# AIGC-Audio/AudioGPT

Measured on AMD Instinct MI355X. Metric: generated audio-seconds/sec (10s clip, 100 DDIM steps) [3 independent batches of 8 prompts in flight per GPU], higher is better.
Workload: dtype bf16x3; 1 GPU; Make-An-Audio T2A batch=8/GPU, 100 DDIM steps, CFG 1.5, UNet+VAE+HiFi-GAN(16k), fp32 storage, bf16x3-split MFMA (hi/lo, fp32 accumulate; meets the fp32 parity gates); prompts_per_gpu=8, ddim_steps=100, mel_frames=624, hipgraph=True, batches_in_flight=3, cfg_lanes=1, concurrency_hint=3, parallelism=prompt-sharded x1 (RCCL bcast cond / gather wav)

## Files before the change

### audiogpt_amd/csrc/ddim.cpp

```cpp
#include "models.h"

#include <cmath>
#include <cstdio>
#include <cstring>

#ifdef MAA_ROCTX
#include <roctracer/roctx.h>
#define MAA_RANGE_PUSH(name) roctxRangePushA(name)
#define MAA_RANGE_POP() roctxRangePop()
#else
#define MAA_RANGE_PUSH(name) ((void)0)
#define MAA_RANGE_POP() ((void)0)
#endif

namespace maa {

namespace {

struct Loop {
    Ctx& ctx;
    UNet& unet;
    const maa_ddim_args& a;
    bool concat, cfg, masked, logging, emb_hoist, share, split;
    int nB, Cin;
// ... 80 lines not shown
        h_step = start;
        MAA_HIP(hipMemcpyAsync(d_step, &h_step, 4, hipMemcpyHostToDevice, ctx.stream));

        if (emb_hoist) unet.emb_table(ctx, tab_t, a.S, emb_tab);

        if (!concat && a.d_cond) {
            if (cfg)
                unet.set_context_cfg(ctx, a.d_uncond, a.d_cond, a.B, a.L, crops);
            else
                unet.set_context(ctx, a.d_cond, nB, a.L, crops);
        }

        const bool two_lanes = cfg && ctx.split_cfg();
        lane2 = two_lanes ? &side_lane(ctx) : nullptr;
        if (lane2 && ctx.prof && !lane2->prof) {
            lane2->prof = new Profiler;
            lane2->prof->detail = ctx.prof->detail;
        }
        share = cfg && emb_hoist && ctx.tune.cfg_shared;
    }

    void prepare() {
        launch_ddim_prepare(ctx, xs, concat ? ccs : nullptr, a.B, nB, per, per_in - per, tab_t, tab_coef, d_step, xin, cur_t,
                            cur_coef, a.d_mask, a.d_x0, a.d_noise_q, a.S, emb_hoist ? emb_tab : nullptr, (int)emb_w, cur_emb, rows);
    }

    void forward() {
        const float* in = xin;
        float* out = eps;
        int h = a.H, w = a.W;
        if (split) {
            launch_split_unfold(ctx, xin, nB, Cin, a.H, a.W, a.split_kh, a.split_kw, a.split_sh, a.split_sw, zin);
            in = zin, out = ecrop, h = a.split_kh, w = a.split_kw;
        }
        const int half = a.B * crops;
        if (lane2) {
            MAA_HIP(hipEventRecord(ctx.ev_fork, ctx.stream));
            MAA_HIP(hipStreamWaitEvent(lane2->stream, ctx.ev_fork, 0));
            unet.forward(ctx, in, cur_t, unet.context_ptr, half, h, w, out, emb_hoist ? cur_emb : nullptr, 0, share ? 2 : 0);
            unet.forward(*lane2, in + (size_t)half * per_crop_in, cur_t + half, unet.context_ptr, half, h, w,
                         out + (size_t)half * per_crop, emb_hoist ? cur_emb : nullptr, half, share ? 3 : 0);
            MAA_HIP(hipEventRecord(ctx.ev_join, lane2->stream));
            MAA_HIP(hipStreamWaitEvent(ctx.stream, ctx.ev_join, 0));
        } else
            unet.forward(ctx, in, cur_t, unet.context_ptr, rows, h, w, out, emb_hoist ? cur_emb : nullptr, -1, share ? 1 : 0);
        if (split)
            launch_split_fold(ctx, ecrop, wT, norm, nB, a.C, a.H, a.W, a.split_kh, a.split_kw, a.split_sh, a.split_sw, eps);
    }

    std::vector<unsigned long long> key(const float* noise_p) const {
        std::vector<unsigned long long> k;
        unet.graph_key(k);
        unsigned scale_bits, temp_bits;
        static_assert(sizeof(scale_bits) == sizeof(a.scale), "float bits");
        std::memcpy(&scale_bits, &a.scale, 4);
        std::memcpy(&temp_bits, &a.temperature, 4);
        k.push_back(temp_bits);
        for (unsigned long long v : {(unsigned long long)a.S, (unsigned long long)a.B, (unsigned long long)a.C, (unsigned long long)a.H,
                                     (unsigned long long)a.W, (unsigned long long)a.Cc, (unsigned long long)a.L,
                                     (unsigned long long)cfg, (unsigned long long)concat, (unsigned long long)scale_bits,
                                     (unsigned long long)ctx.dtype, (unsigned long long)reinterpret_cast<uintptr_t>(slab),
                                     (unsigned long long)reinterpret_cast<uintptr_t>(a.d_mask),
                                     (unsigned long long)reinterpret_cast<uintptr_t>(a.d_x0),
                                     (unsigned long long)reinterpret_cast<uintptr_t>(a.d_noise_q),
                                     (unsigned long long)reinterpret_cast<uintptr_t>(a.h_sigmas ? noise_p : nullptr),
                                     (unsigned long long)reinterpret_cast<uintptr_t>(logging ? a.d_log_x : nullptr),
                                     (unsigned long long)reinterpret_cast<uintptr_t>(logging ? a.d_log_x0 : nullptr),
                                     (unsigned long long)(a.h_sigmas ? 1 : 0),
                                     (unsigned long long)reinterpret_cast<uintptr_t>(ctx.stream),
                                     (unsigned long long)reinterpret_cast<uintptr_t>(ctx.ws.base()),
                                     (unsigned long long)ctx.ws.capacity(),
                                     (unsigned long long)reinterpret_cast<uintptr_t>(lane2 ? lane2->stream : nullptr),
                                     (unsigned long long)reinterpret_cast<uintptr_t>(lane2 ? lane2->ws.base() : nullptr),
                                     (unsigned long long)(lane2 ? lane2->ws.capacity() : 0),
                                     (unsigned long long)a.split_kh, (unsigned long long)a.split_kw, (unsigned long long)a.split_sh,
                                     (unsigned long long)a.split_sw, (unsigned long long)reinterpret_cast<uintptr_t>(wT)})
            k.push_back(v);
        return k;
    }
};

template <class F>
void capture_step(Ctx& ctx, StepGraph& sg, F&& body, std::vector<unsigned long long> key) {
    MAA_HIP(hipStreamBeginCapture(ctx.stream, hipStreamCaptureModeRelaxed));
    try {
        body();
    } catch (...) {
        hipGraph_t dead = nullptr;
        (void)hipStreamEndCapture(ctx.stream, &dead);
        if (dead) (void)hipGraphDestroy(dead);
        throw;
    }
    MAA_HIP(hipStreamEndCapture(ctx.stream, &sg.graph));
    MAA_HIP(hipGraphInstantiate(&sg.exec, sg.graph, nullptr, nullptr, 0));
    sg.key = std::move(key);
}

void ddim_run(Ctx& ctx, UNet& unet, const maa_ddim_args& a, int start, int n_steps, const float* noise_p, float* d_x) {
    MAA_CHECK(a.S > 0 && a.B > 0, "ddim: empty problem");
    MAA_CHECK(start >= 0 && start < a.S && n_steps > 0 && n_steps <= start + 1, "ddim: steps outside the schedule");
    Loop lp(ctx, unet, a, start, d_x);

    auto step_body = [&]() {
        lp.prepare();
        lp.forward();
        launch_ddim_step(ctx, lp.xin, lp.per, lp.per_in, lp.eps, lp.cfg ? lp.eps + a.B * lp.per : nullptr, a.scale, lp.cur_coef,
                         (long long)a.B * lp.per, lp.xs, a.h_sigmas ? noise_p : nullptr, a.temperature, a.S,
                         lp.logging ? a.d_log_x : nullptr, lp.logging ? a.d_log_x0 : nullptr, lp.d_step);
    };

    StepGraph& sg = ctx.ddim_graph;
    int first = 0;
    if (a.use_graph && sg.exec && sg.key == lp.key(noise_p)) {
    } else if (a.use_graph) {
        sg.clear();
        step_body();
        first = 1;
        if (n_steps > 1) capture_step(ctx, sg, step_body, lp.key(noise_p));
    }
    for (int i = first; i < n_steps; ++i) {
#ifdef MAA_ROCTX
        char range[48];
        std::snprintf(range, sizeof(range), "ddim_step %d/%d t=%d", i + 1, n_steps, (int)a.h_timesteps[start - i]);
#endif
        MAA_RANGE_PUSH(range);
        if (a.use_graph)
            MAA_HIP(hipGraphLaunch(sg.exec, ctx.stream));
        else
            step_body();
        MAA_RANGE_POP();
    }
    MAA_HIP(hipMemcpyAsync(d_x, lp.xs, (size_t)a.B * lp.per * 4, hipMemcpyDeviceToDevice, ctx.stream));
    MAA_HIP(hipStreamSynchronize(ctx.stream));
}

}

void ddim_sample(Ctx& ctx, UNet& unet, const maa_ddim_args& a, float* d_x) { ddim_run(ctx, unet, a, a.S - 1, a.S, a.d_noise_p, d_x); }

void ddim_decode(Ctx& ctx, UNet& unet, const maa_ddim_args& a, int t_start, float* d_x) {
    MAA_CHECK(a.S > 0 && a.B > 0, "ddim_decode: empty problem");
    MAA_CHECK(t_start >= 0 && t_start <= a.S, "ddim_decode: t_start must lie in [0, S]");
    MAA_CHECK(!a.d_mask && !a.d_x0 && !a.d_noise_q && !a.h_sqrt_ac && !a.h_sqrt_1mac,
              "ddim_decode: decode has no mask / x0 (ddim.py:243-245)");
    MAA_CHECK(a.n_log == 0 && !a.d_log_x && !a.d_log_x0, "ddim_decode: decode logs no intermediates");
    if (t_start == 0) return;
    const float* noise_p = nullptr;
    if (a.h_sigmas && a.d_noise_p) {
        const long long n = (long long)a.B * a.C * a.H * a.W;
        noise_p = reinterpret_cast<const float*>(reinterpret_cast<uintptr_t>(a.d_noise_p) -
                                                 (uintptr_t)((long long)(a.S - t_start) * n * (long long)sizeof(float)));
    }
    ddim_run(ctx, unet, a, t_start - 1, t_start, noise_p, d_x);
}

void ldm_plms_sample(Ctx& ctx, UNet& unet, const maa_ddim_args& a, float* d_x) {
    MAA_CHECK(a.S > 0 && a.B > 0, "plms: empty problem");
    MAA_CHECK(!a.h_sigmas && !a.d_noise_p, "plms: ddim_eta must be 0 for PLMS (no sigmas, no step noise)");
    Loop lp(ctx, unet, a, a.S - 1, d_x);
    const long long n = (long long)a.B * lp.per;
    float* ring = static_cast<float*>(ctx.plms_ring.get((size_t)3 * n * sizeof(float), ctx.stream));
    const float* eps_c = lp.cfg ? lp.eps + n : nullptr;
    float* log_x = lp.logging ? a.d_log_x : nullptr;
    float* log_x0 = lp.logging ? a.d_log_x0 : nullptr;

    auto euler_step = [&]() {
        lp.prepare();
        lp.forward();
        launch_ldm_plms_euler_mid(ctx, lp.xin, lp.per, lp.per_in, a.B, lp.nB, lp.eps, eps_c, a.scale, lp.cur_coef, lp.xs, ring,
                                  lp.tab_t, lp.cur_t, lp.emb_hoist ? lp.emb_tab : nullptr, (int)lp.emb_w, lp.cur_emb, lp.rows);
        lp.forward();
        launch_ldm_plms_euler_final(ctx, lp.eps, eps_c, a.scale, lp.cur_coef, n, lp.xs, ring, log_x, log_x0, lp.d_step);
    };
    auto ab_step = [&]() {
        lp.prepare();
        lp.forward();
// ... 193 lines not shown
```

### audiogpt_amd/csrc/igemm_dma2.hip

```cpp
#include "igemm_epilogue.h"

#include <cstdio>
#include <cstdlib>
#include <cstring>
#include <type_traits>

namespace maa {

namespace {

template <int BM, int BN, int WGM, int WGN, int NS, int TERMS>
__global__ __launch_bounds__(64 * WGM * WGN) void igemm_dma2_kernel(const IGemm p, int ntiles, int tiles, int Nb,
                                                                     int cps, int items, float* __restrict__ part) {
    constexpr int NW = WGM * WGN, NTH = 64 * NW;
    constexpr int WTM = BM / WGM, WTN = BN / WGN;
    constexpr int MI = WTM / 32, NI = WTN / 32;
    constexpr int ROWS = BM + BN;
    constexpr int STAGE = ROWS * 128;
    constexpr int AI = BM / 8 / NW, BI = BN / 8 / NW;
    constexpr int IPW = AI + BI;
    static_assert(BM % (8 * NW) == 0 && BN % (8 * NW) == 0 && NW % 2 == 0, "copy assignment");
    static_assert(WTM % 32 == 0 && WTN % 32 == 0 && BM % 32 == 0, "tile");
    static_assert(NS >= 3 && (NS - 2) * IPW <= 63, "stages / vmcnt field");
    extern __shared__ __attribute__((aligned(1024))) char smem[];
// ... 157 lines not shown
        }
#pragma unroll
        for (int i = 0; i < MI; ++i)
#pragma unroll
            for (int j = 0; j < NI; ++j) acc[i][j] = __builtin_amdgcn_mfma_f32_32x32x16_bf16(f.ah[i], f.bh[j], acc[i][j], 0, 0, 0);
    };

    int c_w = w_first, c_rem = 0;
    auto item_chunks = [&](int w) __attribute__((always_inline)) {
        const int slice = (w_lo + w) / tiles;
        return min(nchunks, (slice + 1) * cps) - slice * cps;
    };
    auto finish_item = [&]() __attribute__((always_inline)) {
        const int item = w_lo + c_w;
        const int slice = item / tiles, tile = item - slice * tiles;
        const int mt = tile / ntiles, nt = tile - mt * ntiles;
        if (part == nullptr) {
            igemm_epilogue<MI, NI>(p, acc, mt * BM + wm * WTM, nt * BN + wn * WTN, lrow, lk, 0, Nb, rpb);
        } else {
            float* pp = part + ((long long)item * (MI * NI * 4) * NTH + tid) * 4;
#pragma unroll
            for (int i = 0; i < MI; ++i)
#pragma unroll
                for (int j = 0; j < NI; ++j)
#pragma unroll
                    for (int q = 0; q < 4; ++q) {
                        const f32x4 v = {acc[i][j][4 * q], acc[i][j][4 * q + 1], acc[i][j][4 * q + 2], acc[i][j][4 * q + 3]};
                        *reinterpret_cast<f32x4*>(pp + (long long)((i * NI + j) * 4 + q) * NTH * 4) = v;
                    }
        }
        zero_acc();
        c_w += w_step;
        if (c_w >= w_cnt) return false;
        c_rem = item_chunks(c_w);
        return true;
    };

    setup_item(g_w);
    c_rem = item_chunks(c_w);
#pragma unroll
    for (int s = 0; s < NS - 1; ++s) issue(s);

    {
        wait_vmcnt<(NS - 2) * IPW>();
        __builtin_amdgcn_s_barrier();
        Frags f0, f1;
        read_frags(smem, 0, f0);
        int st = 0;
        for (;;) {
            const char* cur = smem + st * STAGE;
            const int st_next = st + 1 == NS ? 0 : st + 1;
            const int st_fill = st == 0 ? NS - 1 : st - 1;
            read_frags(cur, 1, f1);
            __builtin_amdgcn_sched_barrier(0);
            mma(f0);
            __builtin_amdgcn_sched_barrier(0);
            wait_vmcnt<(NS - 3) * IPW>();
            __builtin_amdgcn_s_barrier();
            read_frags(smem + st_next * STAGE, 0, f0);
            __builtin_amdgcn_sched_barrier(0);
            static_for<0, TERMS * MI * NI>([&](auto xc) {
                constexpr int x = decltype(xc)::value;
                constexpr int t = x / (MI * NI) + (3 - TERMS), i = (x % (MI * NI)) / NI, j = x % NI;
                if constexpr (t == 0)
                    acc[i][j] = __builtin_amdgcn_mfma_f32_32x32x16_bf16(f1.al[i], f1.bh[j], acc[i][j], 0, 0, 0);
                else if constexpr (t == 1)
                    acc[i][j] = __builtin_amdgcn_mfma_f32_32x32x16_bf16(f1.ah[i], f1.bl[j], acc[i][j], 0, 0, 0);
                else
                    acc[i][j] = __builtin_amdgcn_mfma_f32_32x32x16_bf16(f1.ah[i], f1.bh[j], acc[i][j], 0, 0, 0);
                if constexpr (x < IPW) copy1(st_fill, xc);
                __builtin_amdgcn_sched_barrier(0);
            });
            if constexpr (IPW > TERMS * MI * NI)
                static_for<TERMS * MI * NI, IPW>([&](auto jc) { copy1(st_fill, jc); });
            advance();
            st = st_next;
            if (--c_rem == 0)
                if (!finish_item()) break;
        }
    }
    wait_vmcnt<0>();
}

template <int JW, int MI, int NI, int WGN, int NTH>
__global__ __launch_bounds__(NTH) void splitk_reduce_kernel(const IGemm p, const float* __restrict__ part, int S, int tiles,
                                                           int ntiles, int Nb) {
    constexpr int njb = NI / JW, nblk = MI * njb;
    constexpr int WTM = 32 * MI, WTN = 32 * NI;
    constexpr int BM = WTM * (NTH / 64 / WGN), BN = WTN * WGN;
    constexpr long long slab = (long long)(MI * NI * 4) * NTH * 4;
    const int tid = threadIdx.x, lane = tid & 63, wid = tid >> 6;
    const int wi = xcd_contiguous((int)blockIdx.x, (int)gridDim.x);
    const int tile = wi / nblk, blk = wi - tile * nblk;
    const int i = blk / njb, j = (blk - i * njb) * JW;
    const int mt = tile / ntiles, nt = tile - mt * ntiles;
    const int wm = wid / WGN, wn = wid - wm * WGN;
    f32x16 acc[1][JW];
#pragma unroll
    for (int jj = 0; jj < JW; ++jj) {
        const float* src = part + (long long)tile * slab + ((long long)((i * NI + j + jj) * 4) * NTH + tid) * 4;
        f32x4 v[4];
#pragma unroll
        for (int q = 0; q < 4; ++q) v[q] = *reinterpret_cast<const f32x4*>(src + (long long)q * NTH * 4);
        for (int s = 1; s < S; ++s) {
            const float* sp = src + (long long)s * tiles * slab;
#pragma unroll
            for (int q = 0; q < 4; ++q) v[q] += *reinterpret_cast<const f32x4*>(sp + (long long)q * NTH * 4);
        }
#pragma unroll
        for (int q = 0; q < 4; ++q)
#pragma unroll
            for (int e = 0; e < 4; ++e) acc[0][jj][4 * q + e] = v[q][e];
    }
    const int rpb = p.Hout * p.Wout;
    igemm_epilogue<1, JW>(p, acc, mt * BM + wm * WTM + i * 32, nt * BN + wn * WTN + j * 32, lane & 31, lane >> 5, 0, Nb, rpb);
}

template <int MI, int NI, int WGN, int NTH>
void launch_reduce_geom(const Ctx& ctx, const IGemm& p, const float* part, int S, int tiles, int ntiles, int Nb) {
    auto go = [&](auto kern, int blocks) {
        hipLaunchKernelGGL(kern, dim3((unsigned)blocks), dim3(NTH), 0, ctx.stream, p, part, S, tiles, ntiles, Nb);
    };
    if (p.geglu) {
        if constexpr (NI % 2 == 0)
            go(splitk_reduce_kernel<2, MI, NI, WGN, NTH>, tiles * MI * (NI / 2));
        else
            MAA_CHECK(false, "split-K reduce: GEGLU needs value / gate block pairs inside a wave");
        return;
    }
    go(splitk_reduce_kernel<1, MI, NI, WGN, NTH>, tiles * MI * NI);
}

template <int BM, int BN, int WGM, int WGN, int NS>
void launch_one(const Ctx& ctx, const IGemm& p, int Nb, int S, float* part) {
    constexpr int NW = WGM * WGN, NTH = 64 * NW;
    constexpr int MI = BM / WGM / 32, NI = BN / WGN / 32;
    const int ncols = p.N * (p.geglu ? 2 : 1);
    const int mtiles = (p.M + BM - 1) / BM, ntiles = (ncols + BN - 1) / BN;
    const int tiles = mtiles * ntiles;
    const int nchunks = p.K / BK;
    const int cps = (nchunks + S - 1) / S;
    const int Seff = (nchunks + cps - 1) / cps;
    MAA_CHECK(Seff == S, "split-K plan leaves an empty slice");
    MAA_CHECK(!p.geglu || NI % 2 == 0, "GEGLU needs value / gate block pairs inside a wave");
    constexpr size_t lds = (size_t)NS * (BM + BN) * 128;
    static_assert(lds <= 163840, "LDS per workgroup");
    const long long items = (long long)tiles * S;
    long long grid = items;
    {
        const int per_cu = (int)(163840 / lds) < 32 / NW ? (int)(163840 / lds) : 32 / NW;
        const long long cap = (long long)device_cu_count(ctx.device) * (per_cu < 1 ? 1 : per_cu);
        if (grid > cap) grid = cap;
    }
    auto go = [&](auto kern) {
        ensure_dynamic_lds(reinterpret_cast<const void*>(kern), ctx.device, (int)lds);
        hipLaunchKernelGGL(kern, dim3((unsigned)grid), dim3(NTH), lds, ctx.stream, p, ntiles, tiles, Nb, cps, (int)items,
                           S > 1 ? part : nullptr);
    };
    if (ctx.dtype == 2)
        go(igemm_dma2_kernel<BM, BN, WGM, WGN, NS, 1>);
    else
        go(igemm_dma2_kernel<BM, BN, WGM, WGN, NS, 3>);
    if (S > 1) launch_splitk_reduce(ctx, p, part, S, tiles, ntiles, Nb, BM, BN, WGN, MI, NI, NTH);
}

}

void launch_splitk_reduce(const Ctx& ctx, const IGemm& p, const float* part, int S, int tiles, int ntiles, int Nb, int BM,
                          int BN, int WGN, int MI, int NI, int NTH) {
    MAA_CHECK(BM == 32 * MI * (NTH / 64 / WGN) && BN == 32 * NI * WGN, "split-K reduce: tile and wave geometry disagree");
    if (MI == 1 && NI == 5 && WGN == 1 && NTH == 512)
        launch_reduce_geom<1, 5, 1, 512>(ctx, p, part, S, tiles, ntiles, Nb);
    else if (MI == 2 && NI == 2 && WGN == 2 && NTH == 512)
        launch_reduce_geom<2, 2, 2, 512>(ctx, p, part, S, tiles, ntiles, Nb);
    else if (MI == 2 && NI == 2 && WGN == 2 && NTH == 256)
        launch_reduce_geom<2, 2, 2, 256>(ctx, p, part, S, tiles, ntiles, Nb);
    else
        MAA_CHECK(false, "split-K reduce: no instantiation for this workgroup geometry");
}

bool igemm_dma2_takes(const Ctx& ctx, const IGemm& p, IGemmPlan& pl) {
    const int ncols = p.N * (p.geglu ? 2 : 1);
    int S = 0;
    if (!ctx.tune.dma2.empty()) {
        if (ctx.tune.dma2 == "off") return false;
        int cfg = 0, ns = 4, pipe = 1, s = 1, kmin = 0, kmax = 1 << 30;
        const int k = std::sscanf(ctx.tune.dma2.c_str(), "%d,%d,%d,%d,%d,%d", &cfg, &ns, &pipe, &s, &kmin, &kmax);
        if (k >= 4) {
            if (p.K < kmin) return false;
            if (p.K <= kmax) S = s < 1 ? 1 : s;
        }
    }
    if (S == 0) {
        if (p.K < 2048 || ncols < 128 || p.geglu) return false;
        S = 2;
    }
    pl.engine = IGemmPlan::DMA2;
    pl.cfg = 0;
    pl.S = fit_slices(p.K / BK, S);
    return true;
}

void launch_igemm_dma2(const Ctx& ctx, const IGemm& p, const IGemmPlan& pl, float* part) {
    MAA_CHECK(pl.S == 1 || part != nullptr, "igemm_dma2: split-K needs its slab workspace");
    launch_one<128, 128, 2, 2, 4>(ctx, p, pl.Nb, pl.S, part);
}

}
```

### audiogpt_amd/csrc/igemm_epilogue.h

```cpp
#pragma once
#include "igemm_device.h"
#include "maa_internal.h"

namespace maa {

__device__ __forceinline__ float fast_erff(float x) {
    const float t = fminf(fabsf(x), 4.0f);
    const float s = t * t;
    float r = -5.654105860e-04f;
    r = fmaf(r, s, 4.923277665e-03f);
    r = fmaf(r, s, -2.671638510e-02f);
    r = fmaf(r, s, 1.128036441e-01f);
    r = fmaf(r, s, -3.761234978e-01f);
    r = fmaf(r, s, 1.128379127e+00f);
    const float small = r * t;
    float q = 1.330939039e-05f;
    q = fmaf(q, t, -3.175720346e-04f);
    q = fmaf(q, t, 3.436867598e-03f);
    q = fmaf(q, t, -2.262198592e-02f);
    q = fmaf(q, t, 1.033189800e-01f);
    q = fmaf(q, t, 6.390933195e-01f);
    q = fmaf(q, t, 1.125925949e+00f);
    q = fmaf(q, t, 7.569686250e-04f);
    const float large = 1.0f - __builtin_amdgcn_exp2f(q * -1.4426950408889634f);
// ... 99 lines not shown
                for (int r = 0; r < 16; ++r) {
                    settle(ra[r]);
                    settle(rs[r]);
                    settle(cv[r]);
                }
                float outv[16];
#pragma unroll
                for (int r = 0; r < 16; ++r) {
                    float v = acc[i][j][r] * p.alpha + bias;
                    if (p.rowadd) v += ra[r];
                    if (resp) v += rs[r];
                    outv[r] = v;
                }
                if (p.act != 0) {
#pragma unroll
                    for (int r = 0; r < 16; ++r) {
                        float v = outv[r];
                        if (p.act == 1) v = tanhf(v);
                        else if (p.act == 2) v = fmaxf(v, 0.f);
                        else if (p.act == 3) v = 0.5f * v * (1.f + fast_erff(v * 0.70710678118654752440f));
                        else if (p.act == 4) v = v > 0.f ? v : v * p.act_slope;
                        outv[r] = v;
                    }
                }
#pragma unroll
                for (int r = 0; r < 16; ++r) {
                    float v = outv[r] * p.out_scale;
                    if (p.accumulate && !p.c_split) v += cv[r];
                    outv[r] = v;
                }
                if constexpr (PAIR) {
                    const bool even = (lrow & 1) == 0;
#pragma unroll
                    for (int rp = 0; rp < 8; ++rp) {
                        const float keep = even ? outv[2 * rp] : outv[2 * rp + 1];
                        const float give = even ? outv[2 * rp + 1] : outv[2 * rp];
                        const float got = __builtin_bit_cast(float, __builtin_amdgcn_update_dpp(0, __builtin_bit_cast(int, give), 0xB1, 0xF, 0xF, false));
                        const int r = 2 * rp + (even ? 0 : 1);
                        const int m = mb + (r & 3) + 8 * (r >> 2) + 4 * lk;
                        if (m < p.M) {
                            const f32x2 v2 = even ? f32x2{keep, got} : f32x2{got, keep};
                            *reinterpret_cast<f32x2*>(cp + (long long)m * p.ldc + (n & ~1)) = v2;
                        }
                    }
                } else {
#pragma unroll
                    for (int r = 0; r < 16; ++r) {
                        const int m = mb + (r & 3) + 8 * (r >> 2) + 4 * lk;
                        if (m < p.M) {
                            if (p.c_split)
                                store_split_pair(cp + (long long)m * p.ldc, n, outv[r]);
                            else
                                cp[(long long)m * p.ldc + n] = outv[r];
                            if (p.c2) {
                                const float w = outv[r] > 0.f ? outv[r] : outv[r] * p.c2_slope;
                                store_split_pair(p.c2 + coff + (long long)m * p.ldc2, n, w);
                            }
                        }
                    }
                }
            }
        }
    }
}

template <int MI, int NI>
__device__ __forceinline__ void igemm_epilogue(const IGemm& p, f32x16 (&acc)[MI][NI], int m_base, int n_base, int lrow,
                                               int lk, long long coff, int Nb, int rpb) {
    const bool pair = !p.geglu && !p.c_split && p.c2 == nullptr && (p.N & 1) == 0 && (p.ldc & 1) == 0 && (coff & 1) == 0 &&
                      (reinterpret_cast<uintptr_t>(p.c) & 7) == 0;
    const bool rsel = !(p.rowadd && rpb < 32);
    if (pair && rsel)
        igemm_epilogue_impl<MI, NI, true, true>(p, acc, m_base, n_base, lrow, lk, coff, Nb, rpb);
    else if (pair)
        igemm_epilogue_impl<MI, NI, true, false>(p, acc, m_base, n_base, lrow, lk, coff, Nb, rpb);
    else if (rsel)
        igemm_epilogue_impl<MI, NI, false, true>(p, acc, m_base, n_base, lrow, lk, coff, Nb, rpb);
    else
        igemm_epilogue_impl<MI, NI, false, false>(p, acc, m_base, n_base, lrow, lk, coff, Nb, rpb);
}

enum class Epi : int { GENERIC = 0, PLAIN = 1, SPLIT = 2, GEGLU = 3 };

inline Epi igemm_epi_kind(const IGemm& p) {
    const bool pitches = p.ldc > 0 && p.ldc < (1 << 24) && p.ldr >= 0 && p.ldr < (1 << 24);
    if (!pitches || p.Z != 1 || p.M <= 0 || p.alpha != 1.f || p.out_scale != 1.f || p.rowadd || p.act != 0 || p.accumulate || p.c2)
        return Epi::GENERIC;
    if (p.geglu) return p.res ? Epi::GENERIC : Epi::GEGLU;
    if (p.c_split) return (p.N & 1) == 0 ? Epi::SPLIT : Epi::GENERIC;
    const bool pair = (p.N & 1) == 0 && (p.ldc & 1) == 0 && (reinterpret_cast<uintptr_t>(p.c) & 7) == 0;
    return pair ? Epi::PLAIN : Epi::GENERIC;
}

__device__ __forceinline__ constexpr unsigned frag_row(int r) { return (unsigned)((r & 3) + 8 * (r >> 2)); }

template <int MI, int NI, Epi KIND, bool FULL, bool RES>
__device__ __forceinline__ void igemm_epilogue_fast_body(const IGemm& p, f32x16 (&acc)[MI][NI], int mb0, int nb0, int lrow, int lk,
                                                         int Nb) {
    const bool even = (lrow & 1) == 0;
    const unsigned ldc = (unsigned)p.ldc, ldr = (unsigned)p.ldr;
    const unsigned lane_f32 = 4u * lk * ldc + lrow;
    const unsigned lane_pair = (4u * lk + (even ? 0u : 1u)) * ldc + (lrow & ~1);
    const unsigned lane_split = 4u * lk * ldc + (lrow >> 1) + (even ? 0u : 16u);
    const unsigned lane_res = 4u * lk * ldr + lrow;
    if constexpr (KIND == Epi::GEGLU) {
        static_assert(NI % 2 == 0, "GEGLU pairs a value block with a gate block");
#pragma unroll
        for (int i = 0; i < MI; ++i) {
            const int mb = mb0 + i * 32;
            if (!FULL && mb >= p.M) break;
#pragma unroll
            for (int j = 0; j < NI; j += 2) {
                const int cb = nb0 + j * 32, ob = (cb >> 6) * 32;
                const int cpk = cb + lrow;
                if (FULL || (cpk + 32 < Nb && ob + lrow < p.N)) {
                    float bv = p.bias ? p.bias[cpk] : 0.f;
                    float bg = p.bias ? p.bias[cpk + 32] : 0.f;
                    settle(bv);
                    settle(bg);
                    float outv[16];
#pragma unroll
                    for (int r = 0; r < 16; ++r) {
                        const float val = acc[i][j][r] + bv;
                        const float g = acc[i][j + 1][r] + bg;
                        const float gl = 0.5f * g * (1.f + fast_erff(g * 0.70710678118654752440f));
                        outv[r] = val * gl;
                    }
                    float* blk = p.c + ((long long)mb * ldc + ob);
                    if (p.c_split) {
#pragma unroll
                        for (int r = 0; r < 16; ++r) {
                            const unsigned w = split_pair_word(even, outv[r]);
                            if (FULL || mb + (int)frag_row(r) + 4 * lk < p.M) reinterpret_cast<unsigned*>(blk)[lane_split + frag_row(r) * ldc] = w;
                        }
                    } else {
#pragma unroll
                        for (int r = 0; r < 16; ++r)
                            if (FULL || mb + (int)frag_row(r) + 4 * lk < p.M) blk[lane_f32 + frag_row(r) * ldc] = outv[r];
                    }
                }
            }
        }
    } else {
#pragma unroll
        for (int i = 0; i < MI; ++i) {
            const int mb = mb0 + i * 32;
            if (!FULL && mb >= p.M) break;
            const unsigned last = (unsigned)(p.M - 1 - mb);
#pragma unroll
            for (int j = 0; j < NI; ++j) {
                const int nb = nb0 + j * 32;
                if (FULL || nb + lrow < p.N) {
                    float bias = p.bias ? p.bias[nb + lrow] : 0.f;
                    float rs[16];
                    if constexpr (RES) {
                        const float* rb = p.res + ((long long)mb * ldr + nb);
#pragma unroll
                        for (int r = 0; r < 16; ++r) {
                            if constexpr (FULL) {
                                rs[r] = rb[lane_res + frag_row(r) * ldr];
                            } else {
                                const unsigned row = frag_row(r) + 4u * lk;
                                rs[r] = rb[(row < last ? row : last) * ldr + lrow];
                            }
                        }
                    }
                    settle(bias);
                    float outv[16];
#pragma unroll
                    for (int r = 0; r < 16; ++r) {
                        float v = acc[i][j][r] + bias;
                        if constexpr (RES) {
                            settle(rs[r]);
                            v += rs[r];
                        }
                        outv[r] = v;
                    }
                    float* blk = p.c + ((long long)mb * ldc + nb);
                    if constexpr (KIND == Epi::PLAIN) {
#pragma unroll
                        for (int rp = 0; rp < 8; ++rp) {
                            const float keep = even ? outv[2 * rp] : outv[2 * rp + 1];
                            const float give = even ? outv[2 * rp + 1] : outv[2 * rp];
                            const float got = __builtin_bit_cast(float, __builtin_amdgcn_update_dpp(0, __builtin_bit_cast(int, give), 0xB1, 0xF, 0xF, false));
                            const f32x2 v2 = even ? f32x2{keep, got} : f32x2{got, keep};
                            if (FULL || mb + (int)frag_row(2 * rp) + 4 * lk + (even ? 0 : 1) < p.M)
                                *reinterpret_cast<f32x2*>(blk + (lane_pair + frag_row(2 * rp) * ldc)) = v2;
                        }
                    } else {
#pragma unroll
                        for (int r = 0; r < 16; ++r) {
                            const unsigned w = split_pair_word(even, outv[r]);
                            if (FULL || mb + (int)frag_row(r) + 4 * lk < p.M) reinterpret_cast<unsigned*>(blk)[lane_split + frag_row(r) * ldc] = w;
                        }
                    }
                }
            }
        }
    }
}

template <int MI, int NI, Epi KIND>
__device__ __forceinline__ void igemm_epilogue_fast(const IGemm& p, f32x16 (&acc)[MI][NI], int m_base, int n_base, int lrow, int lk,
                                                    int Nb) {
    static_assert(KIND != Epi::GENERIC, "the generic kind is igemm_epilogue");
    const int mb0 = __builtin_amdgcn_readfirstlane(m_base), nb0 = __builtin_amdgcn_readfirstlane(n_base);
    if (mb0 >= p.M) return;
    bool full = mb0 + MI * 32 <= p.M;
    if constexpr (KIND == Epi::GEGLU) {
        const int cpk = nb0 + (NI - 2) * 32 + 31;
        if (nb0 + 32 >= Nb) return;
        full = full && cpk + 32 < Nb && (cpk >> 6) * 32 + 31 < p.N;
        if (full)
            igemm_epilogue_fast_body<MI, NI, KIND, true, false>(p, acc, mb0, nb0, lrow, lk, Nb);
        else
            igemm_epilogue_fast_body<MI, NI, KIND, false, false>(p, acc, mb0, nb0, lrow, lk, Nb);
    } else {
        if (nb0 >= p.N) return;
        full = full && nb0 + NI * 32 <= p.N;
        if (p.res) {
            if (full)
                igemm_epilogue_fast_body<MI, NI, KIND, true, true>(p, acc, mb0, nb0, lrow, lk, Nb);
            else
                igemm_epilogue_fast_body<MI, NI, KIND, false, true>(p, acc, mb0, nb0, lrow, lk, Nb);
        } else {
            if (full)
                igemm_epilogue_fast_body<MI, NI, KIND, true, false>(p, acc, mb0, nb0, lrow, lk, Nb);
            else
                igemm_epilogue_fast_body<MI, NI, KIND, false, false>(p, acc, mb0, nb0, lrow, lk, Nb);
        }
    }
}

}
```

### audiogpt_amd/csrc/igemm_pp.hip

```cpp
#include "igemm_epilogue.h"

#include <cstdio>
#include <cstdlib>
#include <type_traits>

namespace maa {

namespace {

constexpr int BM = 256;
constexpr int NSB = 3;

__device__ __forceinline__ void wait_lgkm0() { asm volatile("s_waitcnt lgkmcnt(0)" ::: "memory"); }

struct PPArgs {
    int W, H;
    int T, KW;
    int rowstep, colstep;
    int dh, dw, ph, pw;
    int padflat;
    int NLp;
    int CAPl;
    int ntiles, tiles;
    int items;
// ... 371 lines not shown
    q.NLp = g.NLp;
    q.CAPl = pp_ring_lines(g, BN);
    q.ntiles = ntiles;
    q.tiles = mtiles * ntiles;
    q.nci = p.C1 / BK;
    q.cps = (q.nci + pl.S - 1) / pl.S;
    q.Nb = Nb;
    q.part = pl.S > 1 ? part : nullptr;
    q.S = pl.S;
    q.tile_major = ctx.tune.pp_tile_major && pl.S > 1 ? 1 : 0;
    q.tiles_pp = q.tiles;
    q.b_phase = 0;
    MAA_CHECK((q.nci + q.cps - 1) / q.cps == pl.S, "igemm_pp: K split leaves an empty slice");
    MAA_CHECK(q.CAPl > 0, "igemm_pp: the A ring does not fit beside the weight ring");
    const size_t lds = (size_t)q.CAPl * 128 + (size_t)NSB * BN * 128 + 128 + 1024;
    MAA_CHECK(lds <= 163840, "igemm_pp: LDS per workgroup");
    q.items = q.tiles * pl.S;
    const int cus = device_cu_count(ctx.device);
    const int grid = q.items < cus ? q.items : cus;
    if (g.npa == 1)
        launch_npa<MI, NI, GWM, GWN, 1>(ctx, p, q, grid, lds);
    else
        launch_npa<MI, NI, GWM, GWN, 3>(ctx, p, q, grid, lds);
    if (pl.S > 1) launch_splitk_reduce(ctx, p, part, pl.S, q.tiles, ntiles, Nb, BM, BN, GWN, MI, NI, 512);
}

template <int MI, int NI, int GWM, int GWN>
void launch_up2(const Ctx& ctx, const IGemm& p, int Nb, long long b_phase) {
    constexpr int BN = GWN * NI * 32;
    const int mtiles = (p.M + BM - 1) / BM, ntiles = (p.N + BN - 1) / BN;
    const PPGeom g = pp_geom(p);
    PPArgs q;
    q.W = p.Win;
    q.H = p.Hin;
    q.T = g.T;
    q.KW = g.KW;
    q.rowstep = g.rowstep;
    q.colstep = g.colstep;
    q.dh = p.dh;
    q.dw = p.dw;
    q.ph = 1;
    q.pw = 1;
    q.padflat = p.Win + 1;
    q.NLp = g.NLp;
    q.CAPl = pp_ring_lines(g, BN);
    q.ntiles = ntiles;
    q.tiles_pp = mtiles * ntiles;
    q.tiles = 4 * q.tiles_pp;
    q.nci = p.C1 / BK;
    q.cps = q.nci;
    q.Nb = Nb;
    q.part = nullptr;
    q.S = 1;
    q.tile_major = 0;
    q.b_phase = b_phase;
    MAA_CHECK(q.CAPl > 0, "igemm_pp up2: the A ring does not fit beside the weight ring");
    const size_t lds = (size_t)q.CAPl * 128 + (size_t)NSB * BN * 128 + 128 + 1024;
    MAA_CHECK(lds <= 163840, "igemm_pp up2: LDS per workgroup");
    q.items = q.tiles;
    const int cus = device_cu_count(ctx.device);
    const int grid = q.items < cus ? q.items : cus;
    auto go = [&](auto kern) {
        ensure_dynamic_lds(reinterpret_cast<const void*>(kern), ctx.device, 163840);
        hipLaunchKernelGGL(kern, dim3((unsigned)grid), dim3(512), lds, ctx.stream, p, q);
    };
    const bool one = ctx.dtype == 2;
    if (g.npa == 1) {
        if (one) go(igemm_pp_kernel<MI, NI, GWM, GWN, 1, true, 1, 1, true>);
        else go(igemm_pp_kernel<MI, NI, GWM, GWN, 1, true, 1, 3, true>);
    } else {
        if (one) go(igemm_pp_kernel<MI, NI, GWM, GWN, 3, true, 1, 1, true>);
        else go(igemm_pp_kernel<MI, NI, GWM, GWN, 3, true, 1, 3, true>);
    }
}


struct PP1Args {
    int ntiles, tiles;
    int nchunks, cps;
    int Nb;
    float* part;
};

template <int MI, int NI, int GWM, int GWN, int TERMS>
__global__ __launch_bounds__(512) void igemm_pp1_kernel(const IGemm p, const PP1Args q) {
    constexpr int BN = GWN * NI * 32;
    constexpr int BPG = BN / 16;
    constexpr int NPB = (BPG + 3) / 4;
    constexpr int NPA = 4;
    constexpr int NP = NPA + NPB;
    constexpr int STAGE = (BM + BN) * 128;
    static_assert(GWM * GWN == 4 && GWM * MI * 32 == 128, "group geometry");
    extern __shared__ __attribute__((aligned(1024))) char smem[];
    char* const sD = smem + NSB * STAGE;

    const int tid = threadIdx.x;
    const int lane = tid & 63;
    const int wid = __builtin_amdgcn_readfirstlane(tid >> 6);
    const int grp = wid >> 2, wq = wid & 3;
    const int wm = wq / GWN, wn = wq - wm * GWN;
    const int lrow = lane & 31, lk = lane >> 5;

    const int item = xcd_contiguous((int)blockIdx.x, (int)gridDim.x);
    const int slice = __builtin_amdgcn_readfirstlane(item / q.tiles), tile = item - slice * q.tiles;
    const int mt = __builtin_amdgcn_readfirstlane(tile / q.ntiles), nt = tile - mt * q.ntiles;
    const int m0 = mt * BM, n0 = nt * BN;
    const int c_begin = slice * q.cps;
    const int NQ = min(q.nchunks, c_begin + q.cps) - c_begin;
    const char* const zero = reinterpret_cast<const char*>(p.zeros);

    const int swz = (lrow >> 1) & 7;
    const int a_row = (grp * 128 + wm * (32 * MI) + lrow) * 128, b_row = (BM + wn * (32 * NI) + lrow) * 128;
    int s_off[2][2];
#pragma unroll
    for (int pl = 0; pl < 2; ++pl)
#pragma unroll
        for (int ks = 0; ks < 2; ++ks) s_off[pl][ks] = ((pl * 4 + ks * 2 + lk) ^ swz) << 4;

    const int r8 = lane >> 3, sl = lane & 7;
    const char* gpa[NPA];
    const char* gpb[NPB];
#pragma unroll
    for (int k = 0; k < NPA; ++k) {
        const int rl = 8 * (grp * 16 + k * 4 + wq) + r8;
        const long long m = min((long long)m0 + rl, (long long)p.M - 1);
        gpa[k] = reinterpret_cast<const char*>(p.a1) + (m * p.lda1 + (long long)c_begin * BK) * 4 + ((sl ^ ((rl >> 1) & 7)) << 4);
    }
#pragma unroll
    for (int k = 0; k < NPB; ++k) {
        const int nl = 8 * (grp * BPG + k * 4 + wq) + r8;
        const int n = min(n0 + nl, q.Nb - 1);
        gpb[k] = reinterpret_cast<const char*>(p.b) + ((long long)n * p.ldb + (long long)c_begin * BK) * 4 + ((sl ^ ((nl >> 1) & 7)) << 4);
    }
    auto issue = [&](int slot, bool live) __attribute__((always_inline)) {
        char* const st = smem + slot * STAGE;
        static_for<0, NPA>([&](auto kc) {
            constexpr int k = decltype(kc)::value;
            const char* src = live ? gpa[k] : zero;
            char* dst = live ? st + (grp * 16 + k * 4 + wq) * 1024 : sD;
            __builtin_amdgcn_global_load_lds((gptr_t)src, (lptr_t)dst, 16, 0, 0);
            gpa[k] += 128;
        });
        static_for<0, NPB>([&](auto kc) {
            constexpr int k = decltype(kc)::value;
            const bool real = live && (k * 4 + wq < BPG);
            const char* src = real ? gpb[k] : zero;
            char* dst = real ? st + BM * 128 + (grp * BPG + k * 4 + wq) * 1024 : sD;
            __builtin_amdgcn_global_load_lds((gptr_t)src, (lptr_t)dst, 16, 0, 0);
            gpb[k] += 128;
        });
    };

    issue(0, true);
    issue(1, NQ > 1);
    wait_vmcnt<0>();
    __syncthreads();

    f32x16 acc[MI][NI];
#pragma unroll
    for (int i = 0; i < MI; ++i)
#pragma unroll
        for (int j = 0; j < NI; ++j)
#pragma unroll
            for (int r = 0; r < 16; ++r) acc[i][j][r] = 0.f;
    bf16x8 ah[2][MI], al[2][MI], bh[2][NI], bl[2][NI];

    auto load_phase = [&](int j, int slot) __attribute__((always_inline)) {
        const char* const st = smem + slot * STAGE;
#pragma unroll
        for (int i = 0; i < MI; ++i)
#pragma unroll
            for (int ks = 0; ks < 2; ++ks) {
                ah[ks][i] = *reinterpret_cast<const bf16x8*>(st + a_row + i * 4096 + s_off[0][ks]);
                if constexpr (TERMS == 3) al[ks][i] = *reinterpret_cast<const bf16x8*>(st + a_row + i * 4096 + s_off[1][ks]);
            }
#pragma unroll
        for (int jn = 0; jn < NI; ++jn)
#pragma unroll
            for (int ks = 0; ks < 2; ++ks) {
                bh[ks][jn] = *reinterpret_cast<const bf16x8*>(st + b_row + jn * 4096 + s_off[0][ks]);
                if constexpr (TERMS == 3) bl[ks][jn] = *reinterpret_cast<const bf16x8*>(st + b_row + jn * 4096 + s_off[1][ks]);
            }
        int slot2 = slot + (NSB - 1);
        if (slot2 >= NSB) slot2 -= NSB;
        issue(slot2, j + (NSB - 1) < NQ);
        wait_lgkm0();
        wait_vmcnt<NP>();
    };
    auto mma_phase = [&]() __attribute__((always_inline)) {
#pragma unroll
        for (int ks = 0; ks < 2; ++ks) {
            if constexpr (TERMS == 3) {
#pragma unroll
                for (int i = 0; i < MI; ++i)
#pragma unroll
                    for (int jn = 0; jn < NI; ++jn)
                        acc[i][jn] = __builtin_amdgcn_mfma_f32_32x32x16_bf16(al[ks][i], bh[ks][jn], acc[i][jn], 0, 0, 0);
#pragma unroll
                for (int i = 0; i < MI; ++i)
#pragma unroll
                    for (int jn = 0; jn < NI; ++jn)
                        acc[i][jn] = __builtin_amdgcn_mfma_f32_32x32x16_bf16(ah[ks][i], bl[ks][jn], acc[i][jn], 0, 0, 0);
            }
#pragma unroll
            for (int i = 0; i < MI; ++i)
#pragma unroll
                for (int jn = 0; jn < NI; ++jn)
                    acc[i][jn] = __builtin_amdgcn_mfma_f32_32x32x16_bf16(ah[ks][i], bh[ks][jn], acc[i][jn], 0, 0, 0);
        }
    };

    if (grp == 1) {
        __builtin_amdgcn_sched_barrier(0);
        __builtin_amdgcn_s_barrier();
        __builtin_amdgcn_sched_barrier(0);
    }
    int slot = 0;
    for (int j = 0; j < NQ; ++j) {
        load_phase(j, slot);
        __builtin_amdgcn_sched_barrier(0);
        __builtin_amdgcn_s_barrier();
        __builtin_amdgcn_sched_barrier(0);
        mma_phase();
        __builtin_amdgcn_sched_barrier(0);
        if (!(grp == 1 && j == NQ - 1)) __builtin_amdgcn_s_barrier();
        __builtin_amdgcn_sched_barrier(0);
        if (++slot == NSB) slot = 0;
    }
    wait_vmcnt<0>();

    const int rpb = p.Hout * p.Wout;
    const int row_base = m0 + grp * 128 + wm * (32 * MI), col_base = n0 + wn * (32 * NI);
    if (q.part == nullptr) {
        igemm_epilogue<MI, NI>(p, acc, row_base, col_base, lrow, lk, 0, q.Nb, rpb);
    } else {
        float* pp = q.part + ((long long)item * (MI * NI * 4) * 512 + tid) * 4;
#pragma unroll
        for (int i = 0; i < MI; ++i)
#pragma unroll
            for (int jn = 0; jn < NI; ++jn)
#pragma unroll
                for (int qd = 0; qd < 4; ++qd) {
                    const f32x4 v = {acc[i][jn][4 * qd], acc[i][jn][4 * qd + 1], acc[i][jn][4 * qd + 2], acc[i][jn][4 * qd + 3]};
                    *reinterpret_cast<f32x4*>(pp + (long long)((i * NI + jn) * 4 + qd) * 512 * 4) = v;
                }
    }
}

template <int MI, int NI, int GWM, int GWN>
void launch_one1(const Ctx& ctx, const IGemm& p, const IGemmPlan& pl, float* part) {
    const int Nb = pl.Nb;
    constexpr int BN = GWN * NI * 32;
    const int ncols = p.N * (p.geglu ? 2 : 1);
    const int mtiles = (p.M + BM - 1) / BM, ntiles = (ncols + BN - 1) / BN;
    PP1Args q;
    q.ntiles = ntiles;
    q.tiles = mtiles * ntiles;
    q.nchunks = p.K / BK;
    q.cps = (q.nchunks + pl.S - 1) / pl.S;
    q.Nb = Nb;
    q.part = pl.S > 1 ? part : nullptr;
    MAA_CHECK((q.nchunks + q.cps - 1) / q.cps == pl.S, "igemm_pp: K split leaves an empty slice");
    MAA_CHECK(!p.geglu || NI % 2 == 0, "GEGLU needs value / gate block pairs inside a wave");
    constexpr size_t lds = (size_t)NSB * (BM + BN) * 128 + 1024;
    static_assert(lds <= 163840, "LDS per workgroup");
    const int items = q.tiles * pl.S;
    auto go = [&](auto kern) {
        ensure_dynamic_lds(reinterpret_cast<const void*>(kern), ctx.device, (int)lds);
        hipLaunchKernelGGL(kern, dim3((unsigned)items), dim3(512), lds, ctx.stream, p, q);
    };
    if (ctx.dtype == 2)
        go(igemm_pp1_kernel<MI, NI, GWM, GWN, 1>);
    else
        go(igemm_pp1_kernel<MI, NI, GWM, GWN, 3>);
    if (pl.S > 1) launch_splitk_reduce(ctx, p, part, pl.S, q.tiles, ntiles, Nb, BM, BN, GWN, MI, NI, 512);
}
}

bool igemm_pp_takes(const Ctx& ctx, const IGemm& p, IGemmPlan& pl) {
    const int T = p.KH * p.KW;
    if (!(T >= 3 && T <= 32 && p.sh == 1 && p.sw == 1 && p.up == 0)) return false;
    if (!(2 * p.ph == p.dh * (p.KH - 1) && 2 * p.pw == p.dw * (p.KW - 1))) return false;
    if (!(p.KH == 1 || p.dh * p.Win >= (p.KW - 1) * p.dw)) return false;
    if (!(p.a_split && p.b_split && p.b_nk && p.C2 == 0 && p.C1 % BK == 0 && p.Z == 1 && p.a_act == 0 && !p.geglu)) return false;
    if (p.Hout != p.Hin || p.Wout != p.Win || p.K != T * p.C1 || p.N < 64) return false;
    const PPGeom g = pp_geom(p);
    if (g.npa == 0) return false;
    auto fits = [&](int bn) { return pp_ring_lines(g, bn) > 0; };
    const int nci = p.C1 / BK;
    int bn = 0, S = 0;
    if (!ctx.tune.pp.empty()) {
        if (ctx.tune.pp[0] == 'o') return false;
        std::sscanf(ctx.tune.pp.c_str(), "%d,%d", &bn, &S);
    }
    if (bn != 128 && bn != 160) {
        bn = (p.N % 160 == 0 && fits(160)) ? 160 : 128;
    }
    if (!fits(bn)) {
        if (bn == 160 && fits(128))
            bn = 128;
        else
            return false;
    }
    if (S <= 0) {
        if (p.KH == 1) {
            S = 1;
        } else {
            const int ntiles = (p.N + bn - 1) / bn;
            S = ntiles >= 4 ? ctx.tune.pp_s_wide : ctx.tune.pp_s_narrow;
        }
    }
    pl.engine = IGemmPlan::PP;
    pl.bn = bn;
    pl.S = fit_slices(nci, S);
    return true;
}

void launch_igemm_pp(const Ctx& ctx, const IGemm& p, const IGemmPlan& pl, float* part) {
    MAA_CHECK(pl.bn == 128 || pl.bn == 160, "igemm_pp: problem not planned for this engine");
    MAA_CHECK(pl.S == 1 || part != nullptr, "igemm_pp: split-K needs its slab workspace");
    if (pl.bn == 128)
        launch_one<2, 2, 2, 2>(ctx, p, pl, part);
    else
        launch_one<1, 5, 4, 1>(ctx, p, pl, part);
}


bool launch_igemm_pp_up2(const Ctx& ctx, const IGemm& p, int Nb, long long b_phase) {
    if (ctx.dtype == 0 || (!ctx.tune.pp.empty() && ctx.tune.pp[0] == 'o')) return false;
    if (!(p.KH == 2 && p.KW == 2 && p.sh == 1 && p.sw == 1 && p.dh == 1 && p.dw == 1 && p.up == 0)) return false;
    if (!(p.a_split && p.b_split && p.b_nk && p.C2 == 0 && p.C1 % BK == 0 && p.Z == 1 && p.a_act == 0 && !p.geglu)) return false;
    if (p.Hout != p.Hin || p.Wout != p.Win || p.K != 4 * p.C1 || p.N < 64 || p.C1 / BK < 1) return false;
    const PPGeom g = pp_geom(p);
    if (g.npa == 0) return false;
    int bn = (p.N % 160 == 0 && pp_ring_lines(g, 160) > 0) ? 160 : 128;
    if (pp_ring_lines(g, bn) <= 0) return false;
    if (ctx.ws.dry) return true;
    const int terms = ctx.dtype == 2 ? 1 : 3;
    const char* name = terms == 1 ? (bn == 160 ? "igemm_pp_up2_bf16<256x160>" : "igemm_pp_up2_bf16<256x128>")
                                  : (bn == 160 ? "igemm_pp_up2_bf16x3<256x160>" : "igemm_pp_up2_bf16x3<256x128>");
    ProfScope prof(ctx, name, 2.0 * 4.0 * p.M * (double)p.N * p.K, 4.0 * (4.0 * p.K * p.N + 4.0 * p.M * p.N));
    if (bn == 128)
        launch_up2<2, 2, 2, 2>(ctx, p, Nb, b_phase);
    else
        launch_up2<1, 5, 4, 1>(ctx, p, Nb, b_phase);
    MAA_HIP(hipGetLastError());
    return true;
}

bool igemm_pp1_takes(const Ctx& ctx, const IGemm& p, IGemmPlan& pl) {
    if (!(p.KH == 1 && p.KW == 1 && p.a_split && p.b_split && p.b_nk && p.C2 == 0 && p.Z == 1 && p.a_act == 0 && p.up == 0)) return false;
    if (p.K % BK != 0 || p.K != p.C1 || p.K < 64) return false;
    const int ncols = p.N * (p.geglu ? 2 : 1);
    int bn = 0, S = 0;
    if (!ctx.tune.pp1.empty()) {
        if (ctx.tune.pp1[0] == 'o') return false;
        std::sscanf(ctx.tune.pp1.c_str(), "%d,%d", &bn, &S);
// ... 28 lines not shown
```

Baseline: 146.4 audio-seconds/sec.

## Use specialized fast epilogues in split-K reduce and PP GEMM kernels, add row-add support

The split-K reduce kernel and the igemm_pp1 kernel now dispatch to the templated fast epilogue (PLAIN, SPLIT, GEGLU) instead of always using the generic one. The fast epilogue gains an optional per-batch row-add path so timestep-embedding adds can stay on the fast path. Separately, graph capture now runs on a temporary non-blocking stream rather than the user stream. The aim is to cut epilogue instruction and branch overhead, at the cost of more template instantiations and a more complex row-add boundary split.

```diff
diff --git a/audiogpt_amd/csrc/ddim.cpp b/audiogpt_amd/csrc/ddim.cpp
--- a/audiogpt_amd/csrc/ddim.cpp
+++ b/audiogpt_amd/csrc/ddim.cpp
@@ -186,16 +186,27 @@
 
 template <class F>
 void capture_step(Ctx& ctx, StepGraph& sg, F&& body, std::vector<unsigned long long> key) {
-    MAA_HIP(hipStreamBeginCapture(ctx.stream, hipStreamCaptureModeRelaxed));
-    try {
-        body();
-    } catch (...) {
-        hipGraph_t dead = nullptr;
-        (void)hipStreamEndCapture(ctx.stream, &dead);
-        if (dead) (void)hipGraphDestroy(dead);
-        throw;
-    }
-    MAA_HIP(hipStreamEndCapture(ctx.stream, &sg.graph));
+    hipStream_t const user = ctx.stream;
+    hipStream_t cap = nullptr;
+    MAA_HIP(hipStreamCreateWithFlags(&cap, hipStreamNonBlocking));
+    ctx.stream = cap;
+    hipError_t e = hipStreamBeginCapture(cap, hipStreamCaptureModeRelaxed);
+    if (e == hipSuccess) {
+        try {
+            body();
+        } catch (...) {
+            hipGraph_t dead = nullptr;
+            (void)hipStreamEndCapture(cap, &dead);
+            if (dead) (void)hipGraphDestroy(dead);
+            ctx.stream = user;
+            (void)hipStreamDestroy(cap);
+            throw;
+        }
+        e = hipStreamEndCapture(cap, &sg.graph);
+    }
+    ctx.stream = user;
+    (void)hipStreamDestroy(cap);
+    MAA_HIP(e);
     MAA_HIP(hipGraphInstantiate(&sg.exec, sg.graph, nullptr, nullptr, 0));
     sg.key = std::move(key);
 }
diff --git a/audiogpt_amd/csrc/igemm_dma2.hip b/audiogpt_amd/csrc/igemm_dma2.hip
--- a/audiogpt_amd/csrc/igemm_dma2.hip
+++ b/audiogpt_amd/csrc/igemm_dma2.hip
@@ -263,7 +263,7 @@
     wait_vmcnt<0>();
 }
 
-template <int JW, int MI, int NI, int WGN, int NTH>
+template <int JW, int MI, int NI, int WGN, int NTH, Epi KIND = Epi::GENERIC, bool RADD = false>
 __global__ __launch_bounds__(NTH) void splitk_reduce_kernel(const IGemm p, const float* __restrict__ part, int S, int tiles,
                                                            int ntiles, int Nb) {
     constexpr int njb = NI / JW, nblk = MI * njb;
@@ -294,7 +294,11 @@
             for (int e = 0; e < 4; ++e) acc[0][jj][4 * q + e] = v[q][e];
     }
     const int rpb = p.Hout * p.Wout;
-    igemm_epilogue<1, JW>(p, acc, mt * BM + wm * WTM + i * 32, nt * BN + wn * WTN + j * 32, lane & 31, lane >> 5, 0, Nb, rpb);
+    const int m_base = mt * BM + wm * WTM + i * 32, n_base = nt * BN + wn * WTN + j * 32;
+    if constexpr (KIND == Epi::GENERIC)
+        igemm_epilogue<1, JW>(p, acc, m_base, n_base, lane & 31, lane >> 5, 0, Nb, rpb);
+    else
+        igemm_epilogue_fast<1, JW, KIND, RADD>(p, acc, m_base, n_base, lane & 31, lane >> 5, Nb, 0, rpb);
 }
 
 template <int MI, int NI, int WGN, int NTH>
@@ -302,14 +306,29 @@
     auto go = [&](auto kern, int blocks) {
         hipLaunchKernelGGL(kern, dim3((unsigned)blocks), dim3(NTH), 0, ctx.stream, p, part, S, tiles, ntiles, Nb);
     };
+    Epi kind = ctx.tune.epi_generic ? Epi::GENERIC : igemm_epi_kind(p, true);
+    const bool radd = igemm_epi_rowadd(p);
+    if (radd && kind != Epi::PLAIN) kind = Epi::GENERIC;
     if (p.geglu) {
-        if constexpr (NI % 2 == 0)
-            go(splitk_reduce_kernel<2, MI, NI, WGN, NTH>, tiles * MI * (NI / 2));
-        else
+        if constexpr (NI % 2 == 0) {
+            if (kind == Epi::GEGLU)
+                go(splitk_reduce_kernel<2, MI, NI, WGN, NTH, Epi::GEGLU>, tiles * MI * (NI / 2));
+            else
+                go(splitk_reduce_kernel<2, MI, NI, WGN, NTH>, tiles * MI * (NI / 2));
+        } else {
             MAA_CHECK(false, "split-K reduce: GEGLU needs value / gate block pairs inside a wave");
+        }
         return;
     }
-    go(splitk_reduce_kernel<1, MI, NI, WGN, NTH>, tiles * MI * NI);
+    const int blocks = tiles * MI * NI;
+    if (kind == Epi::PLAIN && radd)
+        go(splitk_reduce_kernel<1, MI, NI, WGN, NTH, Epi::PLAIN, true>, blocks);
+    else if (kind == Epi::PLAIN)
+        go(splitk_reduce_kernel<1, MI, NI, WGN, NTH, Epi::PLAIN>, blocks);
+    else if (kind == Epi::SPLIT)
+        go(splitk_reduce_kernel<1, MI, NI, WGN, NTH, Epi::SPLIT>, blocks);
+    else
+        go(splitk_reduce_kernel<1, MI, NI, WGN, NTH>, blocks);
 }
 
 template <int BM, int BN, int WGM, int WGN, int NS>
diff --git a/audiogpt_amd/csrc/igemm_epilogue.h b/audiogpt_amd/csrc/igemm_epilogue.h
--- a/audiogpt_amd/csrc/igemm_epilogue.h
+++ b/audiogpt_amd/csrc/igemm_epilogue.h
@@ -205,21 +205,23 @@
 
 enum class Epi : int { GENERIC = 0, PLAIN = 1, SPLIT = 2, GEGLU = 3 };
 
-inline Epi igemm_epi_kind(const IGemm& p) {
+inline Epi igemm_epi_kind(const IGemm& p, bool rowadd_ok = false) {
     const bool pitches = p.ldc > 0 && p.ldc < (1 << 24) && p.ldr >= 0 && p.ldr < (1 << 24);
-    if (!pitches || p.Z != 1 || p.M <= 0 || p.alpha != 1.f || p.out_scale != 1.f || p.rowadd || p.act != 0 || p.accumulate || p.c2)
+    if (!pitches || p.Z != 1 || p.M <= 0 || p.alpha != 1.f || p.out_scale != 1.f || p.act != 0 || p.accumulate || p.c2)
         return Epi::GENERIC;
+    if (p.rowadd && !(rowadd_ok && !p.geglu && p.Hout * p.Wout >= 32 && p.ld_rowadd >= 0 && p.ld_rowadd < (1 << 24))) return Epi::GENERIC;
     if (p.geglu) return p.res ? Epi::GENERIC : Epi::GEGLU;
     if (p.c_split) return (p.N & 1) == 0 ? Epi::SPLIT : Epi::GENERIC;
     const bool pair = (p.N & 1) == 0 && (p.ldc & 1) == 0 && (reinterpret_cast<uintptr_t>(p.c) & 7) == 0;
     return pair ? Epi::PLAIN : Epi::GENERIC;
 }
+inline bool igemm_epi_rowadd(const IGemm& p) { return p.rowadd != nullptr; }
 
 __device__ __forceinline__ constexpr unsigned frag_row(int r) { return (unsigned)((r & 3) + 8 * (r >> 2)); }
 
-template <int MI, int NI, Epi KIND, bool FULL, bool RES>
+template <int MI, int NI, Epi KIND, bool FULL, bool RES, bool RADD>
 __device__ __forceinline__ void igemm_epilogue_fast_body(const IGemm& p, f32x16 (&acc)[MI][NI], int mb0, int nb0, int lrow, int lk,
-                                                         int Nb) {
+                                                         int Nb, long long coff, int rpb) {
     const bool even = (lrow & 1) == 0;
     const unsigned ldc = (unsigned)p.ldc, ldr = (unsigned)p.ldr;
     const unsigned lane_f32 = 4u * lk * ldc + lrow;
@@ -249,7 +251,7 @@
                         const float gl = 0.5f * g * (1.f + fast_erff(g * 0.70710678118654752440f));
                         outv[r] = val * gl;
                     }
-                    float* blk = p.c + ((long long)mb * ldc + ob);
+                    float* blk = p.c + (coff + (long long)mb * ldc + ob);
                     if (p.c_split) {
 #pragma unroll
                         for (int r = 0; r < 16; ++r) {
@@ -270,14 +272,29 @@
             const int mb = mb0 + i * 32;
             if (!FULL && mb >= p.M) break;
             const unsigned last = (unsigned)(p.M - 1 - mb);
+            unsigned split = 32u;
+            bool two = false;
+            long long ra_row = 0;
+            if constexpr (RADD) {
+                const int b0 = mb / rpb;
+                split = (unsigned)((b0 + 1) * rpb - mb);
+                two = split < (FULL ? 32u : (last < 31u ? last + 1u : 32u));
+                ra_row = (long long)b0 * p.ld_rowadd;
+            }
 #pragma unroll
             for (int j = 0; j < NI; ++j) {
                 const int nb = nb0 + j * 32;
                 if (FULL || nb + lrow < p.N) {
                     float bias = p.bias ? p.bias[nb + lrow] : 0.f;
+                    float ra_lo = 0.f, ra_hi = 0.f;
+                    if constexpr (RADD) {
+                        const float* ra0 = p.rowadd + (ra_row + nb) + lrow;
+                        ra_lo = ra0[0];
+                        ra_hi = ra0[two ? p.ld_rowadd : 0];
+                    }
                     float rs[16];
                     if constexpr (RES) {
-                        const float* rb = p.res + ((long long)mb * ldr + nb);
+                        const float* rb = p.res + (coff + (long long)mb * ldr + nb);
 #pragma unroll
                         for (int r = 0; r < 16; ++r) {
                             if constexpr (FULL) {
@@ -289,17 +306,22 @@
                         }
                     }
                     settle(bias);
+                    if constexpr (RADD) {
+                        settle(ra_lo);
+                        settle(ra_hi);
+                    }
                     float outv[16];
 #pragma unroll
                     for (int r = 0; r < 16; ++r) {
                         float v = acc[i][j][r] + bias;
+                        if constexpr (RADD) v += frag_row(r) + 4u * lk < split ? ra_lo : ra_hi;
                         if constexpr (RES) {
                             settle(rs[r]);
                             v += rs[r];
                         }
                         outv[r] = v;
                     }
-                    float* blk = p.c + ((long long)mb * ldc + nb);
+                    float* blk = p.c + (coff + (long long)mb * ldc + nb);
                     if constexpr (KIND == Epi::PLAIN) {
 #pragma unroll
                         for (int rp = 0; rp < 8; ++rp) {
@@ -323,10 +345,11 @@
     }
 }
 
-template <int MI, int NI, Epi KIND>
+template <int MI, int NI, Epi KIND, bool RADD = false>
 __device__ __forceinline__ void igemm_epilogue_fast(const IGemm& p, f32x16 (&acc)[MI][NI], int m_base, int n_base, int lrow, int lk,
-                                                    int Nb) {
+                                                    int Nb, long long coff = 0, int rpb = 0) {
     static_assert(KIND != Epi::GENERIC, "the generic kind is igemm_epilogue");
+    static_assert(!(RADD && KIND == Epi::GEGLU), "GEGLU has no row add");
     const int mb0 = __builtin_amdgcn_readfirstlane(m_base), nb0 = __builtin_amdgcn_readfirstlane(n_base);
     if (mb0 >= p.M) return;
     bool full = mb0 + MI * 32 <= p.M;
@@ -335,22 +358,22 @@
         if (nb0 + 32 >= Nb) return;
         full = full && cpk + 32 < Nb && (cpk >> 6) * 32 + 31 < p.N;
         if (full)
-            igemm_epilogue_fast_body<MI, NI, KIND, true, false>(p, acc, mb0, nb0, lrow, lk, Nb);
+            igemm_epilogue_fast_body<MI, NI, KIND, true, false, false>(p, acc, mb0, nb0, lrow, lk, Nb, coff, rpb);
         else
-            igemm_epilogue_fast_body<MI, NI, KIND, false, false>(p, acc, mb0, nb0, lrow, lk, Nb);
+            igemm_epilogue_fast_body<MI, NI, KIND, false, false, false>(p, acc, mb0, nb0, lrow, lk, Nb, coff, rpb);
     } else {
         if (nb0 >= p.N) return;
         full = full && nb0 + NI * 32 <= p.N;
         if (p.res) {
             if (full)
-                igemm_epilogue_fast_body<MI, NI, KIND, true, true>(p, acc, mb0, nb0, lrow, lk, Nb);
+                igemm_epilogue_fast_body<MI, NI, KIND, true, true, RADD>(p, acc, mb0, nb0, lrow, lk, Nb, coff, rpb);
             else
-                igemm_epilogue_fast_body<MI, NI, KIND, false, true>(p, acc, mb0, nb0, lrow, lk, Nb);
+                igemm_epilogue_fast_body<MI, NI, KIND, false, true, RADD>(p, acc, mb0, nb0, lrow, lk, Nb, coff, rpb);
         } else {
             if (full)
-                igemm_epilogue_fast_body<MI, NI, KIND, true, false>(p, acc, mb0, nb0, lrow, lk, Nb);
+                igemm_epilogue_fast_body<MI, NI, KIND, true, false, RADD>(p, acc, mb0, nb0, lrow, lk, Nb, coff, rpb);
             else
-                igemm_epilogue_fast_body<MI, NI, KIND, false, false>(p, acc, mb0, nb0, lrow, lk, Nb);
+                igemm_epilogue_fast_body<MI, NI, KIND, false, false, RADD>(p, acc, mb0, nb0, lrow, lk, Nb, coff, rpb);
         }
     }
 }
diff --git a/audiogpt_amd/csrc/igemm_pp.hip b/audiogpt_amd/csrc/igemm_pp.hip
--- a/audiogpt_amd/csrc/igemm_pp.hip
+++ b/audiogpt_amd/csrc/igemm_pp.hip
@@ -477,7 +477,7 @@
     float* part;
 };
 
-template <int MI, int NI, int GWM, int GWN, int TERMS>
+template <int MI, int NI, int GWM, int GWN, int TERMS, Epi EPI = Epi::GENERIC>
 __global__ __launch_bounds__(512) void igemm_pp1_kernel(const IGemm p, const PP1Args q) {
     constexpr int BN = GWN * NI * 32;
     constexpr int BPG = BN / 16;
@@ -627,7 +627,10 @@
     const int rpb = p.Hout * p.Wout;
     const int row_base = m0 + grp * 128 + wm * (32 * MI), col_base = n0 + wn * (32 * NI);
     if (q.part == nullptr) {
-        igemm_epilogue<MI, NI>(p, acc, row_base, col_base, lrow, lk, 0, q.Nb, rpb);
+        if constexpr (EPI == Epi::GENERIC)
+            igemm_epilogue<MI, NI>(p, acc, row_base, col_base, lrow, lk, 0, q.Nb, rpb);
+        else
+            igemm_epilogue_fast<MI, NI, EPI>(p, acc, row_base, col_base, lrow, lk, q.Nb);
     } else {
         float* pp = q.part + ((long long)item * (MI * NI * 4) * 512 + tid) * 4;
 #pragma unroll
@@ -664,10 +667,23 @@
         ensure_dynamic_lds(reinterpret_cast<const void*>(kern), ctx.device, (int)lds);
         hipLaunchKernelGGL(kern, dim3((unsigned)items), dim3(512), lds, ctx.stream, p, q);
     };
-    if (ctx.dtype == 2)
-        go(igemm_pp1_kernel<MI, NI, GWM, GWN, 1>);
-    else
-        go(igemm_pp1_kernel<MI, NI, GWM, GWN, 3>);
+    auto terms = [&](auto kc) {
+        constexpr Epi K = decltype(kc)::value;
+        if (ctx.dtype == 2)
+            go(igemm_pp1_kernel<MI, NI, GWM, GWN, 1, K>);
+        else
+            go(igemm_pp1_kernel<MI, NI, GWM, GWN, 3, K>);
+    };
+    const Epi kind = q.part != nullptr || ctx.tune.epi_generic ? Epi::GENERIC : igemm_epi_kind(p);
+    if (kind == Epi::PLAIN) {
+        terms(std::integral_constant<Epi, Epi::PLAIN>{});
+    } else if (kind == Epi::SPLIT) {
+        terms(std::integral_constant<Epi, Epi::SPLIT>{});
+    } else if (kind == Epi::GEGLU) {
+        if constexpr (NI % 2 == 0) terms(std::integral_constant<Epi, Epi::GEGLU>{});
+    } else {
+        terms(std::integral_constant<Epi, Epi::GENERIC>{});
+    }
     if (pl.S > 1) launch_splitk_reduce(ctx, p, part, pl.S, q.tiles, ntiles, Nb, BM, BN, GWN, MI, NI, 512);
 }
 }
```

Result: no change. 147.2 audio-seconds/sec (median of 6 runs) (+0.6%).
